# wjwei-handsome/wgatools

Measured on AMD Instinct MI355X. Metric: paf_cigar_ops_per_s (paf2maf+stat), higher is better.
Workload: dtype u8

## Files before the change

wgatools_amd/csrc/capi_paf2maf.inc:

```
static inline u32 job_tiles_for(int param, u64 nt) {
  if (param >= 1) return param > (int)WGA_S_MAX_JOB_TILES ? WGA_S_MAX_JOB_TILES : (u32)param;
  return nt < 200000ull ? 4u : 8u;
}

extern "C" {

size_t wga_tile_ws_bytes(uint64_t n_ops) { return (size_t)(n_tiles(n_ops) * sizeof(wga_tile_sum)) + 16; }

int wga_cigar_stat(wga_ctx* c, const wga_cigar_batch* b, wga_cigar_counts* d_counts,
                   wga_rec_diag* d_diag, void* d_tile_ws) {
  int rc = ctx_bind(c);
  if (rc) return rc;
  if ((rc = check_batch(b))) return rc;
  if (b->n == 0) return WGA_OK;
  if (!d_counts || !d_diag) return fail(WGA_E_INVALID_ARG, "d_counts / d_diag null", nullptr);
  RT_CHECK(rt_memset(d_counts, 0, (size_t)b->n * sizeof(wga_cigar_counts), c->stream));
  RT_CHECK(rt_memset(d_diag, 0xFF, (size_t)b->n * sizeof(wga_rec_diag), c->stream));
  u64 nt = n_tiles(b->n_ops);
  if (nt == 0) return WGA_OK;
  void* ws;
  if ((rc = ctx_scratch(c, (size_t)nt * sizeof(wga_tile_rec), &ws))) return rc;
  wga_tile_rec* tile_rec = (wga_tile_rec*)ws;
  WGA_LAUNCH(k_tile_rec, (u32)((nt + 255) / 256), WGA_BLOCK, c->stream, (const u64*)b->d_op_off,
             b->d_strand_neg, b->n, (u64)b->n_ops, tile_rec);
  LAUNCH_CHECK();
  const u32 grid = (u32)((nt + 3) / 4);
  WGA_LAUNCH(k_cigar_stat, grid, WGA_BLOCK, c->stream, b->d_ops, (const u64*)b->d_op_off,
             b->d_strand_neg, b->n, (u64)b->n_ops, (const wga_tile_rec*)tile_rec, d_counts, d_diag,
             (wga_tile_sum*)d_tile_ws);
  LAUNCH_CHECK();
  return WGA_OK;
}

int wga_exclusive_scan_u64(wga_ctx* c, uint32_t n, const uint64_t* d_in, uint64_t* d_out) {
  int rc = ctx_bind(c);
  if (rc) return rc;
  if (!d_out || (n && !d_in)) return fail(WGA_E_INVALID_ARG, "null array", nullptr);
  ScanPlain f;
  f.in = (const u64*)d_in;
  return run_scan(c, f, n, (u64*)d_out);
}

int wga_paf2maf_layout(wga_ctx* c, uint32_t n, const wga_cigar_counts* d_counts,
                       const uint64_t* d_t_src_len, const uint64_t* d_q_src_len,
                       const uint32_t* d_pre_t, const uint32_t* d_pre_q, const uint32_t* d_post,
                       uint64_t* d_t_row_off, uint64_t* d_q_row_off, uint64_t* d_rec_off) {
  int rc = ctx_bind(c);
  if (rc) return rc;
  if (!d_rec_off) return fail(WGA_E_INVALID_ARG, "d_rec_off null", nullptr);
  if (n && (!d_counts || !d_t_src_len || !d_q_src_len || !d_t_row_off || !d_q_row_off))
    return fail(WGA_E_INVALID_ARG, "null array", nullptr);
  ScanLayout f;
// ... 17 lines not shown
                       const void* d_tile_ws, const uint8_t* d_t_fa, uint64_t t_fa_bytes,
                       const uint64_t* d_t_src_off, const uint64_t* d_t_src_len,
                       const uint8_t* d_q_fa, uint64_t q_fa_bytes, const uint64_t* d_q_src_off,
                       const uint64_t* d_q_src_len, uint8_t* d_out, const uint64_t* d_t_row_off,
                       const uint64_t* d_q_row_off, wga_rec_diag* d_diag) {
  int rc = ctx_bind(c);
  if (rc) return rc;
  if ((rc = check_batch(b))) return rc;
  if (b->n == 0 || b->n_ops == 0) return WGA_OK;
  if (!d_counts || !d_tile_ws || !d_t_src_off || !d_t_src_len || !d_q_src_off || !d_q_src_len ||
      !d_out || !d_t_row_off || !d_q_row_off || !d_diag)
    return fail(WGA_E_INVALID_ARG, "null array", nullptr);
  if ((t_fa_bytes && !d_t_fa) || (q_fa_bytes && !d_q_fa)) return fail(WGA_E_INVALID_ARG, "null sequence pool", nullptr);
  u64 nt = n_tiles(b->n_ops);
  if (nt > 0x7FFFFFFFull) return fail(WGA_E_INVALID_ARG, "batch too large for one launch", nullptr);
  void* ws;
  size_t rec_bytes = ((size_t)b->n * sizeof(wga_rec_desc) + 255) & ~(size_t)255;
  const size_t desc_bytes = (size_t)nt * sizeof(wga_tile_desc);
  const size_t list_bytes = 256 + 2 * (size_t)nt * sizeof(u32);
  const int variant = c->expand_variant >= 0 ? c->expand_variant : WGA_AUTO_LONG_VARIANT;
  c->expand_variant_used = variant;
  const size_t plan_bytes = 0;
  const size_t flag_bytes = variant == 3 ? (((size_t)nt + 255) & ~(size_t)255) : 0;
  if ((rc = ctx_scratch(c, rec_bytes + desc_bytes + list_bytes + plan_bytes + flag_bytes, &ws))) return rc;
  wga_rec_desc* recs = (wga_rec_desc*)ws;
  wga_tile_desc* tdesc = (wga_tile_desc*)((char*)ws + rec_bytes);
  u32* const wide_counts = (u32*)((char*)ws + rec_bytes + desc_bytes);
  u32* const wide_list = wide_counts + 64;
  WGA_LAUNCH(k_rec_desc, (b->n + 255u) / 256u, WGA_BLOCK, c->stream, b->n, d_counts,
             b->d_strand_neg, (const u64*)d_t_src_off, (const u64*)d_t_src_len,
             (const u64*)d_q_src_off, (const u64*)d_q_src_len, (const u64*)d_t_row_off,
             (const u64*)d_q_row_off, recs);
  LAUNCH_CHECK();
  WGA_LAUNCH(k_tile_base, (u32)((nt + 255) / 256), WGA_BLOCK, c->stream, (const u64*)b->d_op_off,
             (u64)b->n_ops, (const wga_tile_sum*)d_tile_ws, (const wga_rec_desc*)recs, tdesc, 0);
  LAUNCH_CHECK();
  ExpandArgs a;
  a.ops = b->d_ops;
  a.op_off = (const u64*)b->d_op_off;
  a.n_ops = b->n_ops;
  a.tdesc = tdesc;
  a.recs = recs;
  a.t_fa = d_t_fa;
  a.t_fa_bytes = t_fa_bytes;
  a.q_fa = d_q_fa;
  a.q_fa_bytes = q_fa_bytes;
  a.out = d_out;
  a.diag = d_diag;
  a.force_slow = c->expand_force_slow;
  a.no_table = c->expand_no_table;
  a.drain_min = 0;
  a.tile_count = nullptr;
  a.tile_list = nullptr;
  a.n_rec = b->n;
  a.job_tiles = job_tiles_for(c->expand_job_tiles, nt);
  const bool stream = variant == 3;
  a.drain_min = c->expand_drain_min ? c->expand_drain_min : ((u64)t_fa_bytes + (u64)q_fa_bytes > WGA_DRAIN_POOL_BYTES ? 16u : 32u);
  c->expand_drain_min_used = a.drain_min;
  u32* const fast_list = wide_list + nt;
  if (stream) {
    u8* const tile_flag = (u8*)ws + rec_bytes + desc_bytes + list_bytes + plan_bytes;
    RT_CHECK(rt_memset(wide_counts, 0, 256, c->stream));
    RT_CHECK(rt_memset(tile_flag, 0, flag_bytes, c->stream));
    WGA_LAUNCH(k_stream_mark_rec, (b->n + 255u) / 256u, WGA_BLOCK, c->stream, b->n, (const wga_rec_desc*)recs,
               (const u64*)b->d_op_off, (u64)t_fa_bytes, (u64)q_fa_bytes, tile_flag);
    LAUNCH_CHECK();
    WGA_LAUNCH(k_stream_mark_tile, (u32)((nt + 255) / 256), WGA_BLOCK, c->stream, tdesc, (u64)nt, (const u8*)tile_flag,
               c->expand_force_slow, wide_counts, fast_list, wide_list);
    LAUNCH_CHECK();
    c->stream_counts = wide_counts;
  }
  const uint32_t slot = c->ev_n % (uint32_t)wga_ctx::kTimingRing;
  if (c->timing) RT_CHECK(rt_event_record(c->ev[2 * slot], c->stream));
  if (stream) {
    const u64 jobs = (nt + a.job_tiles - 1) / a.job_tiles;
    WGA_LAUNCH(k_paf2maf_expand_s, (u32)jobs, 128u, c->stream, a);
    LAUNCH_CHECK();
    const u32 side_grid = nt < 256 ? (u32)nt : 256u;
// ... 66 lines not shown
```

wgatools_amd/csrc/capi_pafpseudo.inc:

```
static CallKey class_tab_key(const wga_cigar_batch* b) {
  return {6, {{b->d_ops, (size_t)b->n_ops * 4}, {b->d_op_off, ((size_t)b->n + 1) * 8}}, {b->n, b->n_ops}};
}

extern "C" {

int wga_cigar_class_sums(wga_ctx* c, const wga_cigar_batch* b, wga_class_sums* d_sums) {
  int rc = ctx_bind(c);
  if (rc) return rc;
  if ((rc = check_batch(b))) return rc;
  if (b->n == 0) return WGA_OK;
  if (!d_sums) return fail(WGA_E_INVALID_ARG, "d_sums null", nullptr);
  wga_ctx::ClassTab& t = c->class_tab;
  const CallKey key = class_tab_key(b);
  t.cache.take(key, false);
  u64 nt = n_tiles(b->n_ops);
  if (nt == 0) {
    RT_CHECK(rt_memset(d_sums, 0, (size_t)b->n * sizeof(wga_class_sums), c->stream));
    return WGA_OK;
  }
  const size_t tile_bytes = ((size_t)nt * sizeof(wga_tile_sum) + 63) & ~(size_t)63;
  const size_t need = tile_bytes + (size_t)b->n * sizeof(wga_class_sums);
  if ((rc = t.buf.reserve(c, need, need + need / 4))) return rc;
  t.tiles = (wga_tile_sum*)t.buf.mem;
  t.rec_sums = (wga_class_sums*)((char*)t.buf.mem + tile_bytes);
// ... 65 lines not shown
  a.q_src_off = (const u64*)d_q_src_off;
  a.q_src_len = (const u64*)d_q_src_len;
  a.skip = (const u64*)d_skip;
  a.out = d_out;
  a.dst_off = (const u64*)d_dst_off;
  a.diag = d_diag;
  a.tile_count = nullptr;
  a.tile_list = nullptr;
  if (stream) {
    char* const base = (char*)ws + tile_bytes + sums_bytes;
    wga_rec_desc* const recs = (wga_rec_desc*)base;
    wga_tile_desc* const tdesc = (wga_tile_desc*)(base + rec_bytes);
    u32* const counts = (u32*)(base + rec_bytes + desc_bytes);
    u32* const list_wide = counts + 64;
    u32* const list_fast = list_wide + nt;
    u8* const tile_flag = (u8*)(base + rec_bytes + desc_bytes + list_bytes);
    RT_CHECK(rt_memset(counts, 0, 256, c->stream));
    RT_CHECK(rt_memset(tile_flag, 0, flag_bytes, c->stream));
    WGA_LAUNCH(k_pseudo_rec_desc, (b->n + 255u) / 256u, WGA_BLOCK, c->stream, b->n, (const wga_class_sums*)rec_sums, b->d_strand_neg,
               base_mode ? (const u64*)d_q_src_off : nullptr, base_mode ? (const u64*)d_q_src_len : nullptr, (const u64*)d_skip,
               (const u64*)d_dst_off, (const u64*)b->d_op_off, (u64)q_fa_bytes, recs, tile_flag);
    LAUNCH_CHECK();
    WGA_LAUNCH(k_tile_base, (u32)((nt + 255) / 256), WGA_BLOCK, c->stream, (const u64*)b->d_op_off, (u64)b->n_ops,
               (const wga_tile_sum*)tiles, (const wga_rec_desc*)recs, tdesc, 1);
    LAUNCH_CHECK();
    WGA_LAUNCH(k_stream_mark_tile, (u32)((nt + 255) / 256), WGA_BLOCK, c->stream, tdesc, (u64)nt, (const u8*)tile_flag, 0, counts,
               list_fast, list_wide);
    LAUNCH_CHECK();
    c->pseudo_counts = counts;
    ExpandArgs e;
    memset(&e, 0, sizeof(e));
    e.ops = b->d_ops;
    e.op_off = (const u64*)b->d_op_off;
    e.n_ops = b->n_ops;
    e.tdesc = tdesc;
    e.recs = recs;
    e.q_fa = base_mode ? d_q_fa : nullptr;
    e.q_fa_bytes = base_mode ? q_fa_bytes : 0;
    e.out = d_out;
    e.diag = d_diag;
    e.n_rec = b->n;
    e.job_tiles = job_tiles_for(c->expand_job_tiles, nt);
    const u64 jobs = (nt + e.job_tiles - 1) / e.job_tiles;
    if (base_mode)
      WGA_LAUNCH(k_pafpseudo_stream, (u32)((jobs + 1) / 2), 128u, c->stream, e);
    else
      WGA_LAUNCH(k_pafpseudo_stream_sym, (u32)((jobs + 1) / 2), 128u, c->stream, e);
// ... 28 lines not shown
```

wgatools_amd/csrc/wga_k_class.h:

```cpp
#ifndef WGA_K_CLASS_H
#define WGA_K_CLASS_H

#include "wga_kernels.h"

__global__ __launch_bounds__(256) void k_class_tiles(const u32* __restrict__ ops,
                                                     const u64* __restrict__ op_off, u32 n,
                                                     u64 n_ops, wga_tile_sum* tiles,
                                                     wga_class_sums* rec_sums) {
  const u32 lane = threadIdx.x & 63u;
  const u32 wave = WGA_WAVE_ID(threadIdx.x);
  const u64 g = (u64)blockIdx.x * 4 + wave;
  const u64 tile_start = g * WGA_TILE;
  if (tile_start >= n_ops) return;
  const u64 tile_end = tile_start + WGA_TILE < n_ops ? tile_start + WGA_TILE : n_ops;
  const u32 nt = (u32)(tile_end - tile_start);
  u32 w[16];
#pragma unroll
  for (int j = 0; j < 4; j++) {
    u32 base = ((u32)j * 64u + lane) * 4u;
    if (base + 3 < nt) {
      u32x4_a16 v = *(const u32x4_a16*)(ops + tile_start + base);
      w[4 * j + 0] = v[0];
      w[4 * j + 1] = v[1];
      w[4 * j + 2] = v[2];
// ... 73 lines not shown
        for (int c = 0; c < 5; c++) f[c] = S[c];
      } else {
#pragma unroll
        for (int c = 0; c < 5; c++)
          if (S[c]) atomicAdd(f + c, S[c]);
      }
    }
#pragma unroll
    for (int c = 0; c < 5; c++) {
      tot[c] += S[c];
      tail[c] = S[c];
    }
    cur = seg_end;
    r++;
  }
  if (tiles && lane == 0) {
    wga_tile_sum ts;
#pragma unroll
    for (int c = 0; c < 5; c++) {
      ts.tot[c] = tot[c];
      ts.tail[c] = tail[c];
    }
    ts.rec = r_first;
    tiles[g] = ts;
  }
}

__global__ __launch_bounds__(256) void k_copy_u64(u64 n, const u64* __restrict__ src, u64* __restrict__ dst) {
  const u64 i = (u64)blockIdx.x * WGA_BLOCK + threadIdx.x;
  if (i < n) dst[i] = src[i];
}

__global__ __launch_bounds__(256) void k_counts_total(u32 n, const u64* __restrict__ counts, u64* totals) {
  const u64 total = (u64)n * 11ull;
  const u64 stride = (u64)gridDim.x * 253ull;
  u64 acc = 0;
  if (threadIdx.x < 253u)
    for (u64 x = (u64)blockIdx.x * 253ull + threadIdx.x; x < total; x += stride) acc += counts[x];
  __shared__ u64 s_acc[256];
  s_acc[threadIdx.x] = threadIdx.x < 253u ? acc : 0ull;
  __syncthreads();
  if (threadIdx.x < 11u) {
    u64 sum = 0;
    for (u32 k = threadIdx.x; k < 253u; k += 11u) sum += s_acc[k];
    if (sum) atomicAdd(totals + threadIdx.x, sum);
  }
// ... 4 lines not shown
```

wgatools_amd/csrc/wga_kernels.h:

```cpp
#ifndef WGA_KERNELS_H
#define WGA_KERNELS_H

#include "../../include/wga_hip.h"
#include "wga_rt.h"

typedef unsigned int u32;
typedef unsigned long long u64;
typedef long long i64;
typedef unsigned char u8;

#define WGA_TILE 1024u
#define WGA_BLOCK 256u
#define WGA_FAST_COL_LIMIT 0x7FFFFFFFull

#define CLS_MX 0u
#define CLS_I 1u
#define CLS_D 2u
#define CLS_S 3u
#define CLS_O 4u

__device__ __forceinline__ u32 op_class(u32 code) {
  const u64 lut = (u64)CLS_MX | ((u64)CLS_I << 3) | ((u64)CLS_D << 6) | ((u64)CLS_O << 9) |
                  ((u64)CLS_S << 12) | ((u64)CLS_O << 15) | ((u64)CLS_O << 18) |
                  ((u64)CLS_MX << 21) | ((u64)CLS_MX << 24) | ((u64)CLS_I << 27) |
                  ((u64)CLS_D << 30) | ((u64)CLS_O << 33) | ((u64)CLS_O << 36) |
                  ((u64)CLS_O << 39) | ((u64)CLS_O << 42) | ((u64)CLS_O << 45);
  return (u32)(lut >> (code * 3)) & 7u;
}

struct wga_tile_sum {
  u64 tot[5];
  u64 tail[5];
  u64 rec;
};

typedef u32 u32x4_a4 __attribute__((vector_size(16), aligned(4)));
typedef u32 u32x4_a16 __attribute__((vector_size(16), aligned(16)));
typedef u32 u32x4_a1 __attribute__((vector_size(16), aligned(1)));

#include <type_traits>

#include "wga_intrin.h"

__device__ __forceinline__ u64 wave_sum_u64(u64 v) {
  for (int m = 32; m >= 1; m >>= 1) v += __shfl_xor(v, m);
  return v;
}


#ifndef WGA_K1_BLOCKS
#define WGA_K1_BLOCKS 5
#endif
#ifndef WGA_K1_WHOLE_TILE_PATH
#define WGA_K1_WHOLE_TILE_PATH 0
#endif
#ifndef WGA_K1_LANE_STORE
#define WGA_K1_LANE_STORE 1
// ... 72 lines not shown
};
__global__ __launch_bounds__(256) void k_tile_rec(const u64* __restrict__ op_off,
                                                  const u8* __restrict__ strand_neg, u32 n, u64 n_ops,
                                                  wga_tile_rec* __restrict__ tile_rec) {
  const u64 g = (u64)blockIdx.x * 256 + threadIdx.x;
  const u64 x = g * WGA_TILE;
  if (x >= n_ops) return;
  u32 lo = 0, hi = n;
  while (hi - lo > 1u) {
    const u32 mid = lo + ((hi - lo) >> 1);
    if (op_off[mid] <= x)
      lo = mid;
    else
      hi = mid;
  }
  wga_tile_rec t;
  t.rec = lo;
  t.neg = strand_neg[lo] != 0 ? 1u : 0u;
  t.rs = op_off[lo];
  t.re = op_off[lo + 1];
  tile_rec[g] = t;
}

__device__ __forceinline__ void cigar_stat_tile(const u64 g, const u32 (&w)[16], const u32 lane, const u64* __restrict__ op_off,
                                                const u8* __restrict__ strand_neg, u64 n_ops,
                                                const wga_tile_rec* __restrict__ tile_rec, wga_cigar_counts* counts,
                                                wga_rec_diag* diag, wga_tile_sum* tiles) {
  const u64 tile_start = g * WGA_TILE;
  const u64 tile_end = tile_start + WGA_TILE < n_ops ? tile_start + WGA_TILE : n_ops;

  const wga_tile_rec tr = tile_rec[g];
  u32 r = WGA_UNI32(tr.rec);
  const u32 r_first = r;
  u64 cur = tile_start;
  u64 tot[5] = {0, 0, 0, 0, 0}, tail[5] = {0, 0, 0, 0, 0};
  u64 re = WGA_UNI64(tr.re);
  constexpr u32 MX_BITS = 0x01810181u, I_BITS = 0x02020202u, X_BITS = 0x01000100u, RARE_BITS = 0xF878F878u;
  constexpr u32 IEV_BITS = 0x00020002u, DEV_BITS = 0x00040004u;
  const u32 lane4 = lane * 4u;
  auto wave_sums = [&](u32 s_mx, u32 s_i, u32 s_t, u32 s_x, u32 ev, u64& Smx, u64& Si, u64& St, u64& Sx, u32& EV) {
    if (__ballot(s_t >= (1u << 26)) == 0ull) {
      Smx = wave_sum_u32(s_mx), Si = wave_sum_u32(s_i), St = wave_sum_u32(s_t), Sx = wave_sum_u32(s_x);
    } else {
      Smx = wave_sum_u32_wide(s_mx), Si = wave_sum_u32_wide(s_i), St = wave_sum_u32_wide(s_t), Sx = wave_sum_u32_wide(s_x);
    }
    EV = wave_sum_u32(ev);
  };
  u64 Wmx, Wi, Wt, Wx;
  u32 Wev;
  bool rare_tile;
  {
    u32 s_mx = 0, s_i = 0, s_t = 0, s_x = 0, ev = 0, rare = 0;
#pragma unroll
    for (int k = 0; k < 16; k++) {
      const u32 op = w[k], len = op >> 4;
      s_mx += len & bit_mask(MX_BITS, op);
      s_i += len & bit_mask(I_BITS, op);
      s_t += len;
      s_x += len & bit_mask(X_BITS, op);
      ev += bit_test(IEV_BITS, op);
      ev += bit_test(DEV_BITS, op) << 16;
      rare |= bit_mask(RARE_BITS, op);
// ... 9 lines not shown
      re = op_off[r + 1];
    }
    const bool first = r == r_first;
    const u64 rs = first ? WGA_UNI64(tr.rs) : op_off[r];
    const bool neg = first ? (WGA_UNI32(tr.neg) != 0u) : (strand_neg[r] != 0);
    const u64 seg_end = re < tile_end ? re : tile_end;
    const u32 a = (u32)(cur - tile_start), b = (u32)(seg_end - tile_start);

    u64 S[5], Sx, St;
    u32 EV, BAD = 0xFFFFFFFFu;
    S[3] = S[4] = 0ull;
    if (!rare_tile && seg_end == tile_end) {
      S[0] = Wmx - Amx, S[1] = Wi - Ai, St = Wt - At, Sx = Wx - Ax;
      EV = Wev - Aev;
    } else {
      const u32 span = b - a;
      u32 s_mx = 0, s_i = 0, s_t = 0, s_s = 0, s_o = 0;
      u32 s_x = 0;
      u32 ev = 0;
      u32 bad = 0xFFFFFFFFu;
      u32 rare = 0;
#pragma unroll
      for (int k = 0; k < 16; k++) {
        const u32 idx = (u32)(k >> 2) * 256u + (u32)(k & 3) + lane4;
        const u32 op = (idx - a < span) ? w[k] : 0u;
        const u32 len = op >> 4;
        s_mx += len & bit_mask(MX_BITS, op);
        s_i += len & bit_mask(I_BITS, op);
        s_t += len;
        s_x += len & bit_mask(X_BITS, op);
        ev += bit_test(IEV_BITS, op);
        ev += bit_test(DEV_BITS, op) << 16;
        rare |= bit_mask(RARE_BITS, op);
      }
      const bool any_rare = rare_tile && __ballot(rare != 0u) != 0ull;
      if (any_rare) {
#pragma unroll
        for (int k = 0; k < 16; k++) {
          const u32 idx = (u32)(k >> 2) * 256u + (u32)(k & 3) + lane4;
          u32 op = (idx - a < span) ? w[k] : 0u;
          WGA_PIN(op);
          const u32 cls = op_class(op & 15u), len = op >> 4;
          s_s += cls == CLS_S ? len : 0u;
          s_o += cls == CLS_O ? len : 0u;
          bad = (cls >= CLS_S && idx < bad) ? idx : bad;
        }
      }
      wave_sums(s_mx, s_i, s_t, s_x, ev, S[0], S[1], St, Sx, EV);
      if (any_rare) {
        S[3] = wave_sum_u32_wide(s_s);
        S[4] = wave_sum_u32_wide(s_o);
        BAD = wave_min_u32(bad);
      }
      Amx += S[0], Ai += S[1], At += St, Ax += Sx, Aev += EV;
    }
    S[2] = St - S[0] - S[1] - S[3] - S[4];
    const u64 Smatch = S[0] - Sx;

#if WGA_K1_LANE_STORE
    {
      const bool whole = rs >= tile_start && re <= tile_end;
      const u64 match = Smatch, mism = S[0] - Smatch;
// ... 59 lines not shown
#pragma unroll
    for (int c = 0; c < 5; c++) {
      tot[c] += S[c];
      tail[c] = S[c];
    }
    cur = seg_end;
    r++;
    if (cur < tile_end) re = op_off[r + 1];
  }
#if WGA_K1_LANE_STORE
  if (tiles) {
    u64 v = 0;
    v = lane_put_u64<0u>(v, tot[0], lane);
    v = lane_put_u64<1u>(v, tot[1], lane);
    v = lane_put_u64<2u>(v, tot[2], lane);
    v = lane_put_u64<3u>(v, tot[3], lane);
    v = lane_put_u64<4u>(v, tot[4], lane);
    v = lane_put_u64<5u>(v, tail[0], lane);
    v = lane_put_u64<6u>(v, tail[1], lane);
    v = lane_put_u64<7u>(v, tail[2], lane);
    v = lane_put_u64<8u>(v, tail[3], lane);
    v = lane_put_u64<9u>(v, tail[4], lane);
    v = lane_put_u64<10u>(v, (u64)r_first, lane);
    if (lane < 11u) ((u64*)(tiles + g))[lane] = v;
  }
#else
  if (tiles && lane == 0) {
    wga_tile_sum ts;
#pragma unroll
    for (int c = 0; c < 5; c++) {
      ts.tot[c] = tot[c];
      ts.tail[c] = tail[c];
    }
    ts.rec = r_first;
    tiles[g] = ts;
  }
#endif
}

__device__ __forceinline__ void stat_load_ops(const u32* __restrict__ ops, u64 n_ops, u64 g, u32 lane, u32 (&w)[16]) {
  const u64 tile_start = g * WGA_TILE;
  const u32 nt = tile_start + WGA_TILE < n_ops ? WGA_TILE : (u32)(n_ops - tile_start);
#pragma unroll
  for (int j = 0; j < 4; j++) {
    const u32 base = ((u32)j * 64u + lane) * 4u;
    u32x4_a16 v = {0u, 0u, 0u, 0u};
    if (base < nt) v = *(const u32x4_a16*)(ops + tile_start + base);
    w[4 * j + 0] = v[0];
    w[4 * j + 1] = v[1];
    w[4 * j + 2] = v[2];
    w[4 * j + 3] = v[3];
  }
  if (nt & 3u) {
#pragma unroll
    for (int k = 0; k < 16; k++) w[k] = ((u32)(k >> 2) * 256u + (u32)(k & 3) + lane * 4u < nt) ? w[k] : 0u;
  }
}

__global__ __launch_bounds__(256, WGA_K1_BLOCKS) void k_cigar_stat(const u32* __restrict__ ops,
                                                    const u64* __restrict__ op_off,
                                                    const u8* __restrict__ strand_neg, u32 n,
                                                    u64 n_ops, const wga_tile_rec* __restrict__ tile_rec,
                                                    wga_cigar_counts* counts,
                                                    wga_rec_diag* diag, wga_tile_sum* tiles) {
  (void)n;
  const u32 lane = threadIdx.x & 63u;
  const u64 g = (u64)blockIdx.x * 4 + WGA_WAVE_ID(threadIdx.x);
  if (g * WGA_TILE >= n_ops) return;
  u32 w[16];
  stat_load_ops(ops, n_ops, g, lane, w);
  cigar_stat_tile(g, w, lane, op_off, strand_neg, n_ops, tile_rec, counts, diag, tiles);
}

__device__ __forceinline__ u64 block_excl_scan_u64(u64 v, u64* s_w , u64* total) {
  const u32 lane = threadIdx.x & 63u, wave = WGA_WAVE_ID(threadIdx.x);
  u64 inc = v;
  for (u32 d = 1; d < 64; d <<= 1) {
    u64 t = __shfl_up(inc, d);
    if (lane >= d) inc += t;
  }
  __syncthreads();
  if (lane == 63) s_w[wave] = inc;
  __syncthreads();
  u64 pre = 0, tot = 0;
  for (u32 k = 0; k < 4; k++) {
    u64 x = s_w[k];
    if (k < wave) pre += x;
    tot += x;
  }
  *total = tot;
  return pre + inc - v;
}

struct ScanPlain {
// ... 586 lines not shown
    case 'T': o = 'A'; break;
    case 'N': o = 'N'; break;
    case 'a': o = 't'; break;
    case 'c': o = 'g'; break;
    case 'g': o = 'c'; break;
    case 't': o = 'a'; break;
    case 'n': o = 'n'; break;
    default:
      o = c;
      atomicMin(bad_base_pos, sidx);
  }
  return o;
}

struct wga_rec_desc {
  u64 t_row_off, q_row_off;
  u64 t_src_off, t_src_len, q_src_off, q_src_len;
  u64 I_total, D_total, L;
  u64 neg;
};
struct wga_tile_base {
  u64 mx, i, d;
};
struct wga_tile_desc {
  u64 tile_cols;
  u32 rec, neg;
  u64 b_mx, b_i, b_d;
  u64 rs, re;
  u64 t_row_off, q_row_off, t_src_off, t_src_len, q_src_off, q_src_len, I_total, D_total, L;
};

__global__ __launch_bounds__(256) void k_rec_desc(u32 n, const wga_cigar_counts* counts,
                                                  const u8* strand_neg, const u64* t_src_off,
                                                  const u64* t_src_len, const u64* q_src_off,
                                                  const u64* q_src_len, const u64* t_row_off,
                                                  const u64* q_row_off, wga_rec_desc* out) {
  u32 r = blockIdx.x * 256u + threadIdx.x;
  if (r >= n) return;
  const wga_cigar_counts cn = counts[r];
  wga_rec_desc d;
  d.t_row_off = t_row_off[r];
  d.q_row_off = q_row_off[r];
  d.t_src_off = t_src_off[r];
  d.t_src_len = t_src_len[r];
  d.q_src_off = q_src_off[r];
  d.q_src_len = q_src_len[r];
  d.I_total = cn.ins_bp + cn.inv_ins_bp;
  d.D_total = cn.del_bp + cn.inv_del_bp;
  d.L = cn.match + cn.mismatch + d.I_total + d.D_total;
  d.neg = (strand_neg[r] != 0 ? 1u : 0u) | (d.t_src_len + d.I_total > d.L ? 2u : 0u) | (d.q_src_len + d.D_total > d.L ? 4u : 0u) |
          ((d.t_src_len + d.I_total < d.L || d.q_src_len + d.D_total < d.L) ? 8u : 0u);
  out[r] = d;
}

__global__ __launch_bounds__(256) void k_tile_base(const u64* op_off, u64 n_ops,
                                                   const wga_tile_sum* tiles,
                                                   const wga_rec_desc* recs, wga_tile_desc* descs, int pseudo) {
  const u32 lane = threadIdx.x & 63u;
  const u64 g = (u64)blockIdx.x * 256 + threadIdx.x;
  const u64 tile_start = g * WGA_TILE;
  const bool valid = tile_start < n_ops;
  wga_tile_sum ts;
  u64 rs = 0, re = 0, g0 = 0;
  if (valid) {
    ts = tiles[g];
    rs = op_off[ts.rec];
    re = op_off[ts.rec + 1];
  }
  u64 p_mx = 0, p_i = 0, p_d = 0;
  bool far = false;
  if (valid && rs < tile_start) {
    g0 = rs / WGA_TILE;
    if (g - g0 <= 64) {
      for (u64 k = g0; k < g; k++) {
        const u64* v = (k == g0) ? tiles[k].tail : tiles[k].tot;
        p_mx += v[CLS_MX];
        p_i += v[CLS_I] + (pseudo ? v[CLS_S] : 0ull);
        p_d += v[CLS_D];
      }
    } else {
// ... 22 lines not shown
    m &= m - 1;
  }
  if (!valid) return;
  const wga_rec_desc rd = recs[ts.rec];
  wga_tile_desc d;
  d.tile_cols = ts.tot[CLS_MX] + ts.tot[CLS_I] + ts.tot[CLS_D] + (pseudo ? ts.tot[CLS_S] : 0ull);
  d.rec = (u32)ts.rec;
  d.neg = (u32)rd.neg;
  d.b_mx = p_mx;
  d.b_i = p_i;
  d.b_d = p_d;
  d.rs = rs;
  d.re = re;
  d.t_row_off = rd.t_row_off;
  d.q_row_off = rd.q_row_off;
  d.t_src_off = rd.t_src_off;
  d.t_src_len = rd.t_src_len;
  d.q_src_off = rd.q_src_off;
  d.q_src_len = rd.q_src_len;
  d.I_total = rd.I_total;
  d.D_total = rd.D_total;
  d.L = rd.L;
  descs[g] = d;
}

struct ExpandArgs {
  const u32* ops;
  const u64* op_off;
  u64 n_ops;
  const wga_tile_desc* tdesc;
  const wga_rec_desc* recs;
  const u8* t_fa;
  u64 t_fa_bytes;
  const u8* q_fa;
  u64 q_fa_bytes;
  u8* out;
  wga_rec_diag* diag;
  int force_slow;
  int no_table;
  u32 drain_min;
  const u32* tile_count;
  const u32* tile_list;
  u32 n_rec;
  u32 job_tiles;
};

#ifndef WGA_K2_BLOCKS
#define WGA_K2_BLOCKS 6
#endif
__device__ __forceinline__ void expand_tile_v1(const ExpandArgs& a, const u64 g) {
  __shared__ u32 s_bnd[3][2];
  __shared__ u32 s_tot[2];
  __shared__ u32 s_tg_col[WGA_TILE + 2];
  __shared__ u32 s_tg_cum[WGA_TILE + 2];
  __shared__ u32 s_qg_col[WGA_TILE + 2];
  __shared__ u32 s_qg_cum[WGA_TILE + 2];
  __shared__ u32 s_zero2[2];
  __shared__ u32 s_w4[16];
  __shared__ u32x4_a16 s_lowmask[17];
  __shared__ u32 s_tbl[WGA_TBL_N + 2];
  __shared__ u32 s_queue[4 * WGA_QCAP];

  const u32 tid = threadIdx.x;
  const u32 lane = tid & 63u, wave = WGA_WAVE_ID(tid);
  const u64 tile_start = g * WGA_TILE;
  const u64 tile_end = tile_start + WGA_TILE < a.n_ops ? tile_start + WGA_TILE : a.n_ops;
  const u32 nt = (u32)(tile_end - tile_start);
// ... 371 lines not shown
```

wgatools_amd/csrc/wga_kernels_k2s.h:

```cpp
#ifndef WGA_KERNELS_K2S_H
#define WGA_KERNELS_K2S_H

#include "wga_kernels.h"

#define WGA_S_FIFO 320u
#define WGA_S_MAX_TILE_COLS (1ull << 24)
#define WGA_S_MAX_JOB_TILES 32u
#define WGA_S_SKIP 0x100u
#define WGA_S_U 4u
#define WGA_S_WAVE_BYTES ((WGA_S_FIFO + 4u) * 8u + 1024u + 1024u + 256u + 272u + 16u)
#ifndef WGA_AUTO_LONG_VARIANT
#define WGA_AUTO_LONG_VARIANT 3
#endif

__global__ __launch_bounds__(256) void k_stream_mark_rec(u32 n, const wga_rec_desc* recs, const u64* op_off, u64 t_fa_bytes,
                                                         u64 q_fa_bytes, u8* tile_flag) {
  const u32 r = blockIdx.x * 256u + threadIdx.x;
  if (r >= n) return;
  const wga_rec_desc d = recs[r];
  const bool inside = d.t_src_off >= 32ull && d.t_src_off + d.t_src_len + 32ull <= t_fa_bytes && d.q_src_off >= 32ull &&
                      d.q_src_off + d.q_src_len + 32ull <= q_fa_bytes;
  if ((d.neg & 0xEull) == 0ull && inside) return;
  const u64 a = op_off[r], b = op_off[r + 1];
  if (b <= a) return;
  for (u64 t = a / WGA_TILE; t <= (b - 1) / WGA_TILE; t++) tile_flag[t] = 1;
}
__global__ __launch_bounds__(256) void k_stream_mark_tile(wga_tile_desc* descs, u64 nt, const u8* tile_flag, int all_slow,
                                                          u32* counts, u32* list_fast, u32* list_slow) {
// ... 72 lines not shown
#define WGA_S_PSEUDO 2
#define WGA_S_SYMBOL 3
template <int MODE>
__device__ __forceinline__ u32 stream_glen(u32 c0, u32 c1) {
  return MODE == WGA_S_SYMBOL ? (c1 >> 1) - (c0 >> 1) : MODE == WGA_S_PSEUDO ? ((int)(c1 - c0) > 0 ? c1 - c0 : 0u) : c1 - c0;
}
__device__ __forceinline__ u32 stream_symbol(u32 cu) { return (cu & 1u) ? 0x2D2D2D2Du : 0x30303030u; }
template <int MODE>
__device__ __forceinline__ void stream_row(const ExpandArgs& a, u8* const lds, const u32 lane, const u64 t0, const u64 t1) {
  u32* const s_fifo = (u32*)lds;
  u32x4_a16* const s_P = (u32x4_a16*)(s_fifo + 2u * (WGA_S_FIFO + 4u));
  u32* const s_q = (u32*)(s_P + 64);
  u32* const s_T = s_q + 256;
  u32x4_a16* const s_lm = (u32x4_a16*)(s_T + 64);
  u64* const s_k = (u64*)(s_lm + 17);
  if (lane < 17u) {
    u32x4_a16 m;
    for (int d = 0; d < 4; d++) m[d] = bytemask(0, (int)lane - 4 * d);
    s_lm[lane] = m;
  }
  constexpr bool QROW = MODE != 0;
  constexpr bool TCOORD = MODE >= WGA_S_PSEUDO;
  constexpr bool SYM = MODE == WGA_S_SYMBOL;
  constexpr u32 COL_MASK = TCOORD ? 0x585u : 0x787u;
  constexpr u32 GAP_MASK = MODE == 0 ? 0x202u : SYM ? 0x504u : 0x404u;
  constexpr u32 SKIP_MASK = MODE == WGA_S_PSEUDO ? 0x212u : 0u;
  const u8* const fa = QROW ? a.q_fa : a.t_fa;
  const u64 fa_bytes = QROW ? a.q_fa_bytes : a.t_fa_bytes;
  const u64 job_lo = t0 * WGA_TILE;
  const u32 q_end = WGA_UNI32((u32)((t1 * WGA_TILE < a.n_ops ? t1 * WGA_TILE : a.n_ops) - job_lo));
  const BufRsrc obuf = buf_make(a.ops + job_lo, (u32)(((a.n_ops - job_lo) < 0x3FFFFFFFull ? (a.n_ops - job_lo) : 0x3FFFFFFFull) * 4ull));

  u32 C_known = 0, cum_known = 0;
  u32 nf = 1;
  u32 e0 = 1;
  u32 pos = 0;
  u32 q = 0;
  u32 q_lo = 0, q_hi = 0;
  u32 rec = 0, re = 0;
  u8* dst_seg = nullptr;
  BufRsrc sbuf = buf_make(fa, 0u);
  u32 S32 = 0;
  bool rc = false;
  bool live = false;
  bool bnd = false;
  bool fin = false;
  u32 C_b = 0, cum_b = 0;
  u32 C_min = 0;
  u64 t = t0;
  u32 ow[4] = {0, 0, 0, 0}, xl0 = 0, xg0 = 0;
  u32 own[4] = {0, 0, 0, 0};

  auto fifo_dedupe = [&]() {
    WGA_WAVE_SYNC();
    u32 n_new = nf;
    if (lane == 0u) {
      u32 w = e0;
      for (u32 r = e0; r < nf; r++) {
        const u32 gs = s_fifo[2u * r], cu = s_fifo[2u * r + 1u];
        const bool dup = w > e0 && s_fifo[2u * (w - 1u)] == gs && (int)(cu - s_fifo[2u * (w - 1u) + 1u]) <= 0 &&
                         (int)(s_fifo[2u * (r + 1u) + 1u] - cu) <= 0;
        if (!dup) {
          s_fifo[2u * w] = gs;
          s_fifo[2u * w + 1u] = cu;
          w++;
        }
      }
      for (u32 k = 0; k < 3u; k++) {
        s_fifo[2u * (w + k)] = s_fifo[2u * (nf + k)];
        s_fifo[2u * (w + k) + 1u] = s_fifo[2u * (nf + k) + 1u];
      }
      n_new = w;
    }
    nf = wave_get_u32(n_new, 0);
// ... 217 lines not shown
            dat[u][3] = pv[3];
          }
          const bool whole = (Ce - Cs) >= 16u && (Cl - Cs) <= wsp2;
          buf_store16_stream(dbuf, whole ? 1024u * u + 16u * lane : WGA_BUF_OOB, dat[u]);
          if (queued && !whole) {
            int lo = (int)(Cs - Cl), hi = (int)(Ce - Cl);
            lo = lo < 0 ? 0 : lo;
            hi = hi > 16 ? 16 : hi;
            stream_store_bytes(B + 1024u * u + lane * 16u, dat[u][0], dat[u][1], dat[u][2], dat[u][3], lo, hi);
          }
        }
        WGA_WAVE_SYNC();
        e0 += nE;
        pos = Ce;
      }
      fin = false;
    }

    if (bnd || !live) {
      const bool sw = bnd;
      u64 row_off, src_off, src_len, x_a, sb;
      bool neg;
      u32 C_a, cum_a;
      if (bnd) {
        const u64 bnd_op = job_lo + re;
        u64 ren;
        do {
          rec++;
          ren = WGA_UNI64(a.op_off[rec + 1]);
        } while (ren <= bnd_op);
        re = ren - job_lo > (u64)q_end ? q_end : (u32)(ren - job_lo);
        const wga_rec_desc* const rd = a.recs + rec;
        row_off = WGA_UNI64(QROW ? rd->q_row_off : rd->t_row_off);
        src_off = WGA_UNI64(QROW ? rd->q_src_off : rd->t_src_off);
        src_len = WGA_UNI64(QROW ? rd->q_src_len : rd->t_src_len);
        neg = (WGA_UNI64(rd->neg) & 1ull) != 0ull;
        x_a = 0;
        sb = 0;
        C_a = C_b;
        cum_a = cum_b;
        if (TCOORD) {
          const u64 skip = WGA_UNI64(rd->t_src_len);
          C_min = C_a + (u32)(skip < 0x40000000ull ? skip : 0x40000000ull);
        }
      } else {
        while (t < t1 && (WGA_UNI32(a.tdesc[t].neg) & WGA_S_SKIP)) t++;
        if (t >= t1) break;
        const wga_tile_desc* const td = a.tdesc + t;
        const u64 tile_start = t * WGA_TILE;
        q = (u32)(tile_start - job_lo);
        WGA_WAVE_SYNC();
        C_known = cum_known = 0u;
        pos = 0u;
        nf = 1u;
        e0 = 1u;
        if (lane < 4u) {
          s_fifo[2u * lane] = 0u;
          s_fifo[2u * lane + 1u] = 0u;
        }
        rec = WGA_UNI32(td->rec);
        const u64 ren = WGA_UNI64(td->re), rs = WGA_UNI64(td->rs);
        re = ren - job_lo > (u64)q_end ? q_end : (u32)(ren - job_lo);
        const bool cont = rs < tile_start;
        const u64 b_mx = cont ? WGA_UNI64(td->b_mx) : 0ull, b_i = cont ? WGA_UNI64(td->b_i) : 0ull,
                  b_d = cont ? WGA_UNI64(td->b_d) : 0ull;
        row_off = WGA_UNI64(QROW ? td->q_row_off : td->t_row_off);
        src_off = WGA_UNI64(QROW ? td->q_src_off : td->t_src_off);
        src_len = WGA_UNI64(QROW ? td->q_src_len : td->t_src_len);
        neg = (WGA_UNI32(td->neg) & 1u) != 0u;
        x_a = TCOORD ? b_mx + b_d : b_mx + b_i + b_d;
        sb = QROW ? b_mx + b_i : b_mx + b_d;
        C_a = cum_a = 0u;
        if (TCOORD) {
          const u64 skip = WGA_UNI64(td->t_src_len);
          const u64 ahead = skip > x_a ? skip - x_a : 0ull;
          C_min = (u32)(ahead < 0x40000000ull ? ahead : 0x40000000ull);
        }
        buf_load16(obuf, q * 4u + lane * 16u, own);
        live = true;
      }
      dst_seg = (u8*)((u64)a.out + row_off + x_a - (u64)C_a);
      rc = QROW && !SYM && neg;
      const u32 adv = C_a - cum_a;
      u64 base;
      if (rc) {
        const u64 top = src_off + src_len;
        const u64 hiB = top > sb ? top - sb : 0ull;
        base = hiB > 0x60000000ull ? hiB - 0x60000000ull : 0ull;
        S32 = (u32)(top - base) - 16u - (u32)sb + adv;
      } else {
        const u64 loB = src_off + sb;
        base = loB > 64ull ? loB - 64ull : 0ull;
        S32 = (u32)(loB - base) - adv;
      }
      base = base > fa_bytes ? fa_bytes : base;
      {
        const u64 left = fa_bytes - base;
        sbuf = buf_make(fa + base, left > 0xFFFFFFF0ull ? 0xFFFFFFF0u : (u32)left);
      }
      if (lane == 0u) s_k[0] = (u64)((i64)sb - (i64)(u64)adv);
      WGA_WAVE_SYNC();
      bnd = false;
      if (sw && re < q_hi) {
        const u32 kb = re - q_lo, e = kb & 3u;
        u32 vl = xl0, vg = xg0;
#pragma unroll
        for (u32 i = 0; i < 3u; i++) {
          const bool valid = q_lo + 4u * lane + i < q_hi && i < e;
          const u32 len = valid ? ow[i] >> 4 : 0u, code = ow[i] & 15u;
          vl += len & bit_mask(COL_MASK, code);
          vg += (len & bit_mask(GAP_MASK, code)) - (len & bit_mask(SKIP_MASK, code));
        }
        C_b = wave_get_u32_dyn(vl, kb >> 2);
        cum_b = wave_get_u32_dyn(vg, kb >> 2);
        bnd = true;
      }
      continue;
    }

    if (q >= q_end) {
      if (pos != C_known) {
        fin = true;
        continue;
      }
      break;
    }
    if ((q & (WGA_TILE - 1u)) == 0u) {
      t = (job_lo + q) / WGA_TILE;
      if (WGA_UNI32(a.tdesc[t].neg) & WGA_S_SKIP) {
        if (pos != C_known) {
          fin = true;
          continue;
        }
        live = false;
        t++;
        continue;
      }
    }
    if (e0 > 1u) {
      const u32 from = e0 - 1u, count = nf + 3u - from;
      for (u32 i0 = 0; i0 < count; i0 += 64u) {
        const u32 i = i0 + lane;
        u64 v = 0;
        if (i < count) v = *(const u64*)(s_fifo + 2u * (from + i));
        WGA_WAVE_SYNC();
        if (i < count) *(u64*)(s_fifo + 2u * i) = v;
        WGA_WAVE_SYNC();
      }
      nf -= from;
      e0 = 1u;
    }
    if (nf + 256u > WGA_S_FIFO) {
      fin = true;
      if (pos != C_known) continue;
      fin = false;
      if (MODE == WGA_S_PSEUDO) {
        fifo_dedupe();
        if (nf + 256u > WGA_S_FIFO) break;
      }
    }
    q_lo = q;
    q_hi = q + 256u < q_end ? q + 256u : q_end;
    q = q_hi;
    ow[0] = own[0], ow[1] = own[1], ow[2] = own[2], ow[3] = own[3];
    buf_load16(obuf, q_hi < q_end ? q_hi * 4u + lane * 16u : WGA_BUF_OOB, own);
    u32 l[4], g[4], sl = 0, sg = 0, sc = 0;
#pragma unroll
    for (int e = 0; e < 4; e++) {
      const bool valid = q_lo + 4u * lane + (u32)e < q_hi;
      const u32 len = valid ? ow[e] >> 4 : 0u, code = ow[e] & 15u;
      l[e] = len & bit_mask(COL_MASK, code);
      g[e] = (len & bit_mask(GAP_MASK, code)) - (len & bit_mask(SKIP_MASK, code));
      sl += l[e];
      sg += g[e];
      sc += g[e] != 0u ? 1u : 0u;
    }
    const u32 il = wave_incl_scan_u32(sl), ig = wave_incl_scan_u32(sg), ic = wave_incl_scan_u32(sc);
    xl0 = C_known + il - sl;
    xg0 = cum_known + ig - sg;
    {
      u32 xl = xl0, xg = xg0, xc = nf + ic - sc;
#pragma unroll
// ... 76 lines not shown
```

Baseline: 80.61 billion.

## Precompute per-tile gap event lists in stat kernel and consume them in expand

The stat kernel gains a variant that, when a tile workspace is supplied, transposes ops through shared memory and writes a per-tile list of insertion and deletion events (column and gap offsets) into the workspace, plus event counts in the tile summary. The streaming expand kernel, for non-pseudo modes, then reads these precomputed events in chunks to fill its FIFO instead of re-scanning every CIGAR op with wave scans. The goal is to move gap discovery out of the expand loop. In exchange, the stat pass does more work, the workspace grows substantially (an 8-byte slot per op), and record-boundary handling is replaced with per-record totals.

```diff
diff --git a/wgatools_amd/csrc/capi_paf2maf.inc b/wgatools_amd/csrc/capi_paf2maf.inc
--- a/wgatools_amd/csrc/capi_paf2maf.inc
+++ b/wgatools_amd/csrc/capi_paf2maf.inc
@@ -5,7 +5,7 @@
 
 extern "C" {
 
-size_t wga_tile_ws_bytes(uint64_t n_ops) { return (size_t)(n_tiles(n_ops) * sizeof(wga_tile_sum)) + 16; }
+size_t wga_tile_ws_bytes(uint64_t n_ops) { return (size_t)(WGA_EV_OFFSET(n_tiles(n_ops)) + n_tiles(n_ops) * (u64)WGA_EV_SLOT); }
 
 int wga_cigar_stat(wga_ctx* c, const wga_cigar_batch* b, wga_cigar_counts* d_counts,
                    wga_rec_diag* d_diag, void* d_tile_ws) {
@@ -25,9 +25,14 @@
              b->d_strand_neg, b->n, (u64)b->n_ops, tile_rec);
   LAUNCH_CHECK();
   const u32 grid = (u32)((nt + 3) / 4);
-  WGA_LAUNCH(k_cigar_stat, grid, WGA_BLOCK, c->stream, b->d_ops, (const u64*)b->d_op_off,
-             b->d_strand_neg, b->n, (u64)b->n_ops, (const wga_tile_rec*)tile_rec, d_counts, d_diag,
-             (wga_tile_sum*)d_tile_ws);
+  if (d_tile_ws)
+    WGA_LAUNCH(k_cigar_stat_ev, grid, WGA_BLOCK, c->stream, b->d_ops, (const u64*)b->d_op_off,
+               b->d_strand_neg, b->n, (u64)b->n_ops, (const wga_tile_rec*)tile_rec, d_counts, d_diag,
+               (wga_tile_sum*)d_tile_ws, (u8*)d_tile_ws + WGA_EV_OFFSET(nt));
+  else
+    WGA_LAUNCH(k_cigar_stat, grid, WGA_BLOCK, c->stream, b->d_ops, (const u64*)b->d_op_off,
+               b->d_strand_neg, b->n, (u64)b->n_ops, (const wga_tile_rec*)tile_rec, d_counts, d_diag,
+               (wga_tile_sum*)nullptr);
   LAUNCH_CHECK();
   return WGA_OK;
 }
@@ -91,7 +96,9 @@
   c->expand_variant_used = variant;
   const size_t plan_bytes = 0;
   const size_t flag_bytes = variant == 3 ? (((size_t)nt + 255) & ~(size_t)255) : 0;
-  if ((rc = ctx_scratch(c, rec_bytes + desc_bytes + list_bytes + plan_bytes + flag_bytes, &ws))) return rc;
+  const size_t tev_bytes = variant == 3 ? (size_t)nt * sizeof(wga_tile_ev) : 0;
+  if ((rc = ctx_scratch(c, rec_bytes + desc_bytes + list_bytes + plan_bytes + flag_bytes + tev_bytes, &ws))) return rc;
+  wga_tile_ev* const tev = variant == 3 ? (wga_tile_ev*)((char*)ws + rec_bytes + desc_bytes + list_bytes + plan_bytes + flag_bytes) : nullptr;
   wga_rec_desc* recs = (wga_rec_desc*)ws;
   wga_tile_desc* tdesc = (wga_tile_desc*)((char*)ws + rec_bytes);
   u32* const wide_counts = (u32*)((char*)ws + rec_bytes + desc_bytes);
@@ -102,7 +109,7 @@
              (const u64*)d_q_row_off, recs);
   LAUNCH_CHECK();
   WGA_LAUNCH(k_tile_base, (u32)((nt + 255) / 256), WGA_BLOCK, c->stream, (const u64*)b->d_op_off,
-             (u64)b->n_ops, (const wga_tile_sum*)d_tile_ws, (const wga_rec_desc*)recs, tdesc, 0);
+             (u64)b->n_ops, (const wga_tile_sum*)d_tile_ws, (const wga_rec_desc*)recs, tdesc, 0, tev);
   LAUNCH_CHECK();
   ExpandArgs a;
   a.ops = b->d_ops;
@@ -123,6 +130,8 @@
   a.tile_list = nullptr;
   a.n_rec = b->n;
   a.job_tiles = job_tiles_for(c->expand_job_tiles, nt);
+  a.tev = tev;
+  a.events = (const u8*)d_tile_ws + WGA_EV_OFFSET(nt);
   const bool stream = variant == 3;
   a.drain_min = c->expand_drain_min ? c->expand_drain_min : ((u64)t_fa_bytes + (u64)q_fa_bytes > WGA_DRAIN_POOL_BYTES ? 16u : 32u);
   c->expand_drain_min_used = a.drain_min;
diff --git a/wgatools_amd/csrc/capi_pafpseudo.inc b/wgatools_amd/csrc/capi_pafpseudo.inc
--- a/wgatools_amd/csrc/capi_pafpseudo.inc
+++ b/wgatools_amd/csrc/capi_pafpseudo.inc
@@ -111,7 +111,7 @@
                (const u64*)d_dst_off, (const u64*)b->d_op_off, (u64)q_fa_bytes, recs, tile_flag);
     LAUNCH_CHECK();
     WGA_LAUNCH(k_tile_base, (u32)((nt + 255) / 256), WGA_BLOCK, c->stream, (const u64*)b->d_op_off, (u64)b->n_ops,
-               (const wga_tile_sum*)tiles, (const wga_rec_desc*)recs, tdesc, 1);
+               (const wga_tile_sum*)tiles, (const wga_rec_desc*)recs, tdesc, 1, (wga_tile_ev*)nullptr);
     LAUNCH_CHECK();
     WGA_LAUNCH(k_stream_mark_tile, (u32)((nt + 255) / 256), WGA_BLOCK, c->stream, tdesc, (u64)nt, (const u8*)tile_flag, 0, counts,
                list_fast, list_wide);
diff --git a/wgatools_amd/csrc/wga_k_class.h b/wgatools_amd/csrc/wga_k_class.h
--- a/wgatools_amd/csrc/wga_k_class.h
+++ b/wgatools_amd/csrc/wga_k_class.h
@@ -119,6 +119,7 @@
       ts.tail[c] = tail[c];
     }
     ts.rec = r_first;
+    ts.ev = 0;
     tiles[g] = ts;
   }
 }
diff --git a/wgatools_amd/csrc/wga_kernels.h b/wgatools_amd/csrc/wga_kernels.h
--- a/wgatools_amd/csrc/wga_kernels.h
+++ b/wgatools_amd/csrc/wga_kernels.h
@@ -32,7 +32,10 @@
   u64 tot[5];
   u64 tail[5];
   u64 rec;
+  u64 ev;
 };
+#define WGA_EV_SLOT (8u * WGA_TILE)
+#define WGA_EV_OFFSET(n_tiles) (((u64)(n_tiles) * sizeof(wga_tile_sum) + 16ull + 255ull) & ~255ull)
 
 typedef u32 u32x4_a4 __attribute__((vector_size(16), aligned(4)));
 typedef u32 u32x4_a16 __attribute__((vector_size(16), aligned(16)));
@@ -151,10 +154,12 @@
   tile_rec[g] = t;
 }
 
+template <bool EVT>
 __device__ __forceinline__ void cigar_stat_tile(const u64 g, const u32 (&w)[16], const u32 lane, const u64* __restrict__ op_off,
                                                 const u8* __restrict__ strand_neg, u64 n_ops,
                                                 const wga_tile_rec* __restrict__ tile_rec, wga_cigar_counts* counts,
-                                                wga_rec_diag* diag, wga_tile_sum* tiles) {
+                                                wga_rec_diag* diag, wga_tile_sum* tiles, u8* events = nullptr,
+                                                u64* s_ev = nullptr ) {
   const u64 tile_start = g * WGA_TILE;
   const u64 tile_end = tile_start + WGA_TILE < n_ops ? tile_start + WGA_TILE : n_ops;
 
@@ -166,7 +171,7 @@
   u64 re = WGA_UNI64(tr.re);
   constexpr u32 MX_BITS = 0x01810181u, I_BITS = 0x02020202u, X_BITS = 0x01000100u, RARE_BITS = 0xF878F878u;
   constexpr u32 IEV_BITS = 0x00020002u, DEV_BITS = 0x00040004u;
-  const u32 lane4 = lane * 4u;
+  const u32 lane4 = EVT ? lane * 16u : lane * 4u;
   auto wave_sums = [&](u32 s_mx, u32 s_i, u32 s_t, u32 s_x, u32 ev, u64& Smx, u64& Si, u64& St, u64& Sx, u32& EV) {
     if (__ballot(s_t >= (1u << 26)) == 0ull) {
       Smx = wave_sum_u32(s_mx), Si = wave_sum_u32(s_i), St = wave_sum_u32(s_t), Sx = wave_sum_u32(s_x);
@@ -222,7 +227,7 @@
       u32 rare = 0;
 #pragma unroll
       for (int k = 0; k < 16; k++) {
-        const u32 idx = (u32)(k >> 2) * 256u + (u32)(k & 3) + lane4;
+        const u32 idx = (EVT ? (u32)k : (u32)(k >> 2) * 256u + (u32)(k & 3)) + lane4;
         const u32 op = (idx - a < span) ? w[k] : 0u;
         const u32 len = op >> 4;
         s_mx += len & bit_mask(MX_BITS, op);
@@ -237,7 +242,7 @@
       if (any_rare) {
 #pragma unroll
         for (int k = 0; k < 16; k++) {
-          const u32 idx = (u32)(k >> 2) * 256u + (u32)(k & 3) + lane4;
+          const u32 idx = (EVT ? (u32)k : (u32)(k >> 2) * 256u + (u32)(k & 3)) + lane4;
           u32 op = (idx - a < span) ? w[k] : 0u;
           WGA_PIN(op);
           const u32 cls = op_class(op & 15u), len = op >> 4;
@@ -343,7 +348,44 @@
     v = lane_put_u64<8u>(v, tail[3], lane);
     v = lane_put_u64<9u>(v, tail[4], lane);
     v = lane_put_u64<10u>(v, (u64)r_first, lane);
-    if (lane < 11u) ((u64*)(tiles + g))[lane] = v;
+    if (!EVT && lane < 12u) ((u64*)(tiles + g))[lane] = v;
+    if (EVT) {
+      constexpr u32 COL_BITS = 0x07870787u, D_BITS = 0x04040404u;
+      u32 c = 0, gi = 0, gd = 0, n = 0;
+#pragma unroll
+      for (int k = 0; k < 16; k++) {
+        const u32 op = w[k], len = op >> 4;
+        const u32 li = len & bit_mask(I_BITS, op), ld = len & bit_mask(D_BITS, op);
+        c += len & bit_mask(COL_BITS, op);
+        gi += li;
+        gd += ld;
+        n += (li != 0u ? 1u : 0u) + (ld != 0u ? 0x10000u : 0u);
+      }
+      const u32 ic = wave_incl_scan_u32(c), ii = wave_incl_scan_u32(gi), id = wave_incl_scan_u32(gd), in = wave_incl_scan_u32(n);
+      v = lane_put_u64<11u>(v, (u64)wave_last_u32(in), lane);
+      if (lane < 12u) ((u64*)(tiles + g))[lane] = v;
+      u32 xc = ic - c, xi = ii - gi, xd = id - gd;
+      u32 kt = (in - n) & 0xFFFFu;
+      u32 kq = WGA_TILE - 1u - ((in - n) >> 16);
+      WGA_WAVE_SYNC();
+#pragma unroll
+      for (int k = 0; k < 16; k++) {
+        const u32 op = w[k], len = op >> 4;
+        const u32 li = len & bit_mask(I_BITS, op), ld = len & bit_mask(D_BITS, op);
+        if (li != 0u) s_ev[kt++] = (u64)xc | ((u64)xi << 32);
+        if (ld != 0u) s_ev[kq--] = (u64)xc | ((u64)xd << 32);
+        xc += len & bit_mask(COL_BITS, op);
+        xi += li;
+        xd += ld;
+      }
+      WGA_WAVE_SYNC();
+      const u32 nev = wave_last_u32(in);
+      const u32 pt = ((nev & 0xFFFFu) + 1u) >> 1, pq = ((nev >> 16) + 1u) >> 1;
+      const u32x4_a16* const img = (const u32x4_a16*)s_ev;
+      u32x4_a16* const slot = (u32x4_a16*)events;
+      for (u32 i = lane; i < pt; i += 64u) slot[i] = img[i];
+      for (u32 i = lane; i < pq; i += 64u) slot[WGA_TILE / 2u - 1u - i] = img[WGA_TILE / 2u - 1u - i];
+    }
   }
 #else
   if (tiles && lane == 0) {
@@ -354,8 +396,10 @@
       ts.tail[c] = tail[c];
     }
     ts.rec = r_first;
+    ts.ev = 0;
     tiles[g] = ts;
   }
+  static_assert(!EVT, "the event lists need WGA_K1_LANE_STORE");
 #endif
 }
 
@@ -390,7 +434,37 @@
   if (g * WGA_TILE >= n_ops) return;
   u32 w[16];
   stat_load_ops(ops, n_ops, g, lane, w);
-  cigar_stat_tile(g, w, lane, op_off, strand_neg, n_ops, tile_rec, counts, diag, tiles);
+  cigar_stat_tile<false>(g, w, lane, op_off, strand_neg, n_ops, tile_rec, counts, diag, tiles);
+}
+#ifndef WGA_K1_EV_BLOCKS
+#define WGA_K1_EV_BLOCKS 4
+#endif
+__global__ __launch_bounds__(256, WGA_K1_EV_BLOCKS) void k_cigar_stat_ev(const u32* __restrict__ ops,
+                                                    const u64* __restrict__ op_off,
+                                                    const u8* __restrict__ strand_neg, u32 n,
+                                                    u64 n_ops, const wga_tile_rec* __restrict__ tile_rec,
+                                                    wga_cigar_counts* counts,
+                                                    wga_rec_diag* diag, wga_tile_sum* tiles, u8* events) {
+  (void)n;
+  __shared__ u32x4_a16 s_tp[4][WGA_TILE / 2u];
+  const u32 lane = threadIdx.x & 63u, wave = WGA_WAVE_ID(threadIdx.x);
+  const u64 g = (u64)blockIdx.x * 4 + wave;
+  if (g * WGA_TILE >= n_ops) return;
+  u32 w[16];
+  stat_load_ops(ops, n_ops, g, lane, w);
+#pragma unroll
+  for (int j = 0; j < 4; j++) {
+    const u32x4_a16 v = {w[4 * j], w[4 * j + 1], w[4 * j + 2], w[4 * j + 3]};
+    s_tp[wave][(u32)j * 64u + lane] = v;
+  }
+  WGA_WAVE_SYNC();
+#pragma unroll
+  for (int j = 0; j < 4; j++) {
+    const u32x4_a16 v = s_tp[wave][lane * 4u + (u32)j];
+    w[4 * j] = v[0], w[4 * j + 1] = v[1], w[4 * j + 2] = v[2], w[4 * j + 3] = v[3];
+  }
+  cigar_stat_tile<true>(g, w, lane, op_off, strand_neg, n_ops, tile_rec, counts, diag, tiles, events + g * (u64)WGA_EV_SLOT,
+                        (u64*)s_tp[wave]);
 }
 
 __device__ __forceinline__ u64 block_excl_scan_u64(u64 v, u64* s_w , u64* total) {
@@ -1023,6 +1097,9 @@
 struct wga_tile_base {
   u64 mx, i, d;
 };
+struct wga_tile_ev {
+  u32 cols, gap_t, gap_q, n;
+};
 struct wga_tile_desc {
   u64 tile_cols;
   u32 rec, neg;
@@ -1056,7 +1133,8 @@
 
 __global__ __launch_bounds__(256) void k_tile_base(const u64* op_off, u64 n_ops,
                                                    const wga_tile_sum* tiles,
-                                                   const wga_rec_desc* recs, wga_tile_desc* descs, int pseudo) {
+                                                   const wga_rec_desc* recs, wga_tile_desc* descs, int pseudo,
+                                                   wga_tile_ev* tev) {
   const u32 lane = threadIdx.x & 63u;
   const u64 g = (u64)blockIdx.x * 256 + threadIdx.x;
   const u64 tile_start = g * WGA_TILE;
@@ -1125,6 +1203,14 @@
   d.D_total = rd.D_total;
   d.L = rd.L;
   descs[g] = d;
+  if (tev) {
+    wga_tile_ev e;
+    e.cols = (u32)d.tile_cols;
+    e.gap_t = (u32)ts.tot[CLS_I];
+    e.gap_q = (u32)ts.tot[CLS_D];
+    e.n = (u32)ts.ev;
+    tev[g] = e;
+  }
 }
 
 struct ExpandArgs {
@@ -1146,6 +1232,8 @@
   const u32* tile_list;
   u32 n_rec;
   u32 job_tiles;
+  const wga_tile_ev* tev;
+  const u8* events;
 };
 
 #ifndef WGA_K2_BLOCKS
diff --git a/wgatools_amd/csrc/wga_kernels_k2s.h b/wgatools_amd/csrc/wga_kernels_k2s.h
--- a/wgatools_amd/csrc/wga_kernels_k2s.h
+++ b/wgatools_amd/csrc/wga_kernels_k2s.h
@@ -4,6 +4,7 @@
 #include "wga_kernels.h"
 
 #define WGA_S_FIFO 320u
+#define WGA_S_EV_CHUNK 128u
 #define WGA_S_MAX_TILE_COLS (1ull << 24)
 #define WGA_S_MAX_JOB_TILES 32u
 #define WGA_S_SKIP 0x100u
@@ -122,6 +123,8 @@
   constexpr bool QROW = MODE != 0;
   constexpr bool TCOORD = MODE >= WGA_S_PSEUDO;
   constexpr bool SYM = MODE == WGA_S_SYMBOL;
+  constexpr bool EVT = MODE < WGA_S_PSEUDO;
+  constexpr u32 CHUNK = EVT ? WGA_S_EV_CHUNK : 256u;
   constexpr u32 COL_MASK = TCOORD ? 0x585u : 0x787u;
   constexpr u32 GAP_MASK = MODE == 0 ? 0x202u : SYM ? 0x504u : 0x404u;
   constexpr u32 SKIP_MASK = MODE == WGA_S_PSEUDO ? 0x212u : 0u;
@@ -150,6 +153,26 @@
   u64 t = t0;
   u32 ow[4] = {0, 0, 0, 0}, xl0 = 0, xg0 = 0;
   u32 own[4] = {0, 0, 0, 0};
+  const BufRsrc ebuf = buf_make(EVT ? a.events + t0 * (u64)WGA_EV_SLOT : nullptr, EVT ? (u32)(t1 - t0) * WGA_EV_SLOT : 0u);
+  u32 ek = 0, ne = 0;
+  bool tin = false;
+  u32 bC = 0, bG = 0, tC = 0, tG = 0;
+  u32 ewn[4] = {0, 0, 0, 0};
+  bool has_b = false;
+  auto ev_request = [&](const u64 tt, const u32 k) {
+    const u32 slot = (u32)(tt - t0) * WGA_EV_SLOT;
+    const u32 off = QROW ? slot + WGA_EV_SLOT - 8u * k - 16u * (lane + 1u) : slot + 8u * k + 16u * lane;
+    buf_load16(ebuf, tt < t1 ? off : WGA_BUF_OOB, ewn);
+  };
+  auto ev_tile = [&]() {
+    const wga_tile_ev* const te = a.tev + t;
+    const u32 n = WGA_UNI32(te->n);
+    ne = QROW ? n >> 16 : n & 0xFFFFu;
+    tC = bC + WGA_UNI32(te->cols);
+    tG = bG + WGA_UNI32(QROW ? te->gap_q : te->gap_t);
+    ek = 0u;
+    tin = false;
+  };
 
   auto fifo_dedupe = [&]() {
     WGA_WAVE_SYNC();
@@ -413,6 +436,7 @@
       u64 row_off, src_off, src_len, x_a, sb;
       bool neg;
       u32 C_a, cum_a;
+      u64 c_left = 0, g_left = 0;
       if (bnd) {
         const u64 bnd_op = job_lo + re;
         u64 ren;
@@ -430,6 +454,10 @@
         sb = 0;
         C_a = C_b;
         cum_a = cum_b;
+        if (EVT) {
+          c_left = WGA_UNI64(rd->L);
+          g_left = WGA_UNI64(QROW ? rd->D_total : rd->I_total);
+        }
         if (TCOORD) {
           const u64 skip = WGA_UNI64(rd->t_src_len);
           C_min = C_a + (u32)(skip < 0x40000000ull ? skip : 0x40000000ull);
@@ -467,7 +495,15 @@
           const u64 ahead = skip > x_a ? skip - x_a : 0ull;
           C_min = (u32)(ahead < 0x40000000ull ? ahead : 0x40000000ull);
         }
-        buf_load16(obuf, q * 4u + lane * 16u, own);
+        if (EVT) {
+          c_left = WGA_UNI64(td->L) - x_a;
+          g_left = WGA_UNI64(QROW ? td->D_total : td->I_total) - (QROW ? b_d : b_i);
+          bC = bG = 0u;
+          ev_tile();
+          ev_request(t, 0u);
+        } else {
+          buf_load16(obuf, q * 4u + lane * 16u, own);
+        }
         live = true;
       }
       dst_seg = (u8*)((u64)a.out + row_off + x_a - (u64)C_a);
@@ -492,7 +528,12 @@
       if (lane == 0u) s_k[0] = (u64)((i64)sb - (i64)(u64)adv);
       WGA_WAVE_SYNC();
       bnd = false;
-      if (sw && re < q_hi) {
+      if (EVT) {
+        has_b = re < q_end && c_left < 0x40000000ull;
+        C_b = C_a + (u32)c_left;
+        cum_b = cum_a + (u32)g_left;
+        bnd = has_b && (int)(C_known - C_b) >= 0;
+      } else if (sw && re < q_hi) {
         const u32 kb = re - q_lo, e = kb & 3u;
         u32 vl = xl0, vg = xg0;
 #pragma unroll
@@ -509,14 +550,37 @@
       continue;
     }
 
-    if (q >= q_end) {
+    if (EVT) {
+      if (tin) {
+        const u64 tn = t + 1u;
+        if (tn >= t1) {
+          if (pos != C_known) {
+            fin = true;
+            continue;
+          }
+          break;
+        }
+        if (WGA_UNI32(a.tdesc[tn].neg) & WGA_S_SKIP) {
+          if (pos != C_known) {
+            fin = true;
+            continue;
+          }
+          live = false;
+          t = tn + 1u;
+          continue;
+        }
+        t = tn;
+        bC = tC;
+        bG = tG;
+        ev_tile();
+      }
+    } else if (q >= q_end) {
       if (pos != C_known) {
         fin = true;
         continue;
       }
       break;
-    }
-    if ((q & (WGA_TILE - 1u)) == 0u) {
+    } else if ((q & (WGA_TILE - 1u)) == 0u) {
       t = (job_lo + q) / WGA_TILE;
       if (WGA_UNI32(a.tdesc[t].neg) & WGA_S_SKIP) {
         if (pos != C_known) {
@@ -541,14 +605,53 @@
       nf -= from;
       e0 = 1u;
     }
-    if (nf + 256u > WGA_S_FIFO) {
+    if (nf + CHUNK > WGA_S_FIFO) {
       fin = true;
       if (pos != C_known) continue;
       fin = false;
       if (MODE == WGA_S_PSEUDO) {
         fifo_dedupe();
-        if (nf + 256u > WGA_S_FIFO) break;
-      }
+        if (nf + CHUNK > WGA_S_FIFO) break;
+      }
+    }
+    if (EVT) {
+      const u32 rem = ne - ek;
+      const bool last = rem <= WGA_S_EV_CHUNK;
+      const u32 cnt = last ? rem : WGA_S_EV_CHUNK - 1u;
+      u32 sC = tC, sG = tG;
+      if (rem != 0u) {
+        const u32 c0 = ewn[QROW ? 2 : 0] + bC, g0 = ewn[QROW ? 3 : 1] + bG;
+        const u32 c1 = ewn[QROW ? 0 : 2] + bC, g1 = ewn[QROW ? 1 : 3] + bG;
+        const u32 i0 = 2u * lane;
+        if (i0 < cnt) {
+          s_fifo[2u * (nf + i0)] = c0;
+          s_fifo[2u * (nf + i0) + 1u] = g0;
+        }
+        if (i0 + 1u < cnt) {
+          s_fifo[2u * (nf + i0) + 2u] = c1;
+          s_fifo[2u * (nf + i0) + 3u] = g1;
+        }
+        if (!last) {
+          sC = wave_get_u32(c1, 63);
+          sG = wave_get_u32(g1, 63);
+        }
+      }
+      ek += cnt;
+      tin = last;
+      nf += cnt;
+      C_known = sC;
+      cum_known = sG;
+      if (lane < 3u) {
+        s_fifo[2u * (nf + lane)] = C_known;
+        s_fifo[2u * (nf + lane) + 1u] = cum_known;
+      }
+      if (!last)
+        ev_request(t, ek);
+      else if (t + 1u < t1)
+        ev_request(t + 1u, 0u);
+      WGA_WAVE_SYNC();
+      bnd = has_b && (int)(C_known - C_b) >= 0;
+      continue;
     }
     q_lo = q;
     q_hi = q + 256u < q_end ? q + 256u : q_end;
```

New measurement: 82.34 billion (median of 6 runs). 1.02x the previous value.
